# CliffKai/BridgeLang

Hardware: AMD Instinct MI355X
Metric: action-seqs/sec (7-DoF, 224px) openvla-7b bf16 (higher is better)
Workload: dtype bf16; 1 GPU; openvla-7b bf16 inference (BASELINE configs[1]): batch 16 synthetic 224px frames + 32-token prompts per GPU, predict_action = vision towers + projector + Llama prefill S=288 + 6 cached decode steps, greedy; 7 batches in flight: per step one batch is submitted (vision+prefill) while decode iteration g of the batch submitted g steps earlier, g = 1..6, runs as ONE merged 96-row pass over the weights ; batch_per_gpu=16, prompt_len=32, seq_len=288, replicas=1, hip_graph=True, pipeline_depth=7

## Files before the change

### bridgelang_amd/csrc/gemm_bf16.hip

```cpp
#include "gemm_common.h"
#include <stdlib.h>

namespace bl_gemm_bf16_impl {
using namespace blgemm;

typedef __attribute__((ext_vector_type(4))) short s16x4_t;

template <int EPI>
__global__ __launch_bounds__(256) void gemm128_kernel(GemmArgs p) {
#if defined(__HIP_DEVICE_COMPILE__)
  constexpr int BM = 128, BN = 128, WN = 2, NWAVE = 4;
  constexpr int TM = 64, TN = 64, MT = 4, NT = 4;
  constexpr int A_BYTES = BM * ROW_BYTES, BUF_BYTES = A_BYTES + BN * ROW_BYTES;
  extern __shared__ __attribute__((aligned(16))) char smem[];

  int tm, tn;
  tile_coords(p, tm, tn);
  const int m0 = tm * BM, n0 = tn * BN;
  const int tid = threadIdx.x, lane = tid & 63;
  const int wave = __builtin_amdgcn_readfirstlane(tid >> 6);
  const int wm = wave / WN, wn = wave % WN;
  const int kt32 = p.K >> 5;

  const unsigned a_bytes = (unsigned)min((long)p.M * p.lda * 2, 0xffffffffL);
// ... 631 lines not shown
  constexpr int A_BYTES = BM * ROW_BYTES, DUMMY = A_BYTES, W_OFF = A_BYTES + 4096, STAGE = W_OFF + 32768;
  extern __shared__ __attribute__((aligned(16))) char smem[];
  int tm, tn;
  tile_coords(p, tm, tn);
  const int m0 = tm * BM, n0 = tn * BN;
  const int tid = threadIdx.x, lane = tid & 63;
  const int wave = __builtin_amdgcn_readfirstlane(tid >> 6);
  const int wm = wave >> 2, wn = wave & 3;
  const int l15 = lane & 15, lg = lane >> 4;
  const int kt32 = p.K >> 5, nk = p.K / BK;

  const unsigned a_bytes = (unsigned)min((long)p.M * p.lda * 2, 0xffffffffL);
  const unsigned w_bytes = (unsigned)min((long)p.N * p.K * 2, 0xffffffffL);
  const int prow = lane >> 3, pchunk = (lane & 7) ^ prow;
  unsigned voffA[5];
  int ldsA[5];
#pragma unroll
  for (int j = 0; j < 5; ++j) {
    const int pi = wave + 8 * j;
    voffA[j] = (unsigned)(((long)(m0 + pi * 8 + prow) * p.lda) * 2 + pchunk * 16);
    ldsA[j] = pi < 36 ? pi * 1024 : DUMMY + (pi - 36) * 1024;
  }
  const unsigned a4_bytes = wave < 4 ? a_bytes : 0u;
  unsigned voffW[2];
#pragma unroll
  for (int q = 0; q < 2; ++q) voffW[q] = (unsigned)((long)(n0 / 16 + 2 * wave + q) * kt32 * 1024 + lane * 16);
  const int ldsW = W_OFF + 2 * wave * 2048;
#define BL_RS(PTR, BYTES) __builtin_amdgcn_make_buffer_rsrc((void*)(PTR), 0, (BYTES), 0x00020000)
#define ISSUE_A(J, TILE)                                                                                  \
  do {                                                                                                    \
    const int t__ = (TILE);                                                                               \
    const __amdgpu_buffer_rsrc_t rs__ = BL_RS(p.A, t__ < nk ? ((J) < 4 ? a_bytes : a4_bytes) : 0u);       \
    BL_GLDS(rs__, smem + (t__ & 1) * STAGE + ldsA[J], voffA[J], t__ * 128);                               \
  } while (0)
#define ISSUE_W(Q, KS, TILE)                                                                              \
  do {                                                                                                    \
    const int t__ = (TILE);                                                                               \
    const __amdgpu_buffer_rsrc_t rs__ = BL_RS(p.W, t__ < nk ? w_bytes : 0u);                              \
    BL_GLDS(rs__, smem + (t__ & 1) * STAGE + ldsW + (Q) * 2048 + (KS) * 1024, voffW[Q] + (KS) * 1024, t__ * 2048); \
  } while (0)
  const int cb0 = (lg ^ (lane & 7)) << 4;
  const int offX = (wm * 144 + l15) * ROW_BYTES;
  const int offY = W_OFF + wn * 8192 + lane * 16;
#define READ_X(T3, SB)                                                                                    \
  _Pragma("unroll") for (int i = 0; i < 3; ++i) {                                                         \
    X[i * 2] = *(const bf16x8_t*)((SB) + offX + (3 * (T3) + i) * 2048 + cb0);                             \
    X[i * 2 + 1] = *(const bf16x8_t*)((SB) + offX + (3 * (T3) + i) * 2048 + (cb0 ^ 64));                  \
  }
#define READ_Y(DST, NH, SB)                                                                               \
  _Pragma("unroll") for (int j = 0; j < 2; ++j) {                                                         \
    DST[j * 2] = *(const bf16x8_t*)((SB) + offY + (2 * (NH) + j) * 2048);                                 \
    DST[j * 2 + 1] = *(const bf16x8_t*)((SB) + offY + (2 * (NH) + j) * 2048 + 1024);                      \
  }
#define MMA(YR, T3, NH)                                                                                   \
  _Pragma("unroll") for (int ks = 0; ks < 2; ++ks)                                                        \
    _Pragma("unroll") for (int j = 0; j < 2; ++j)                                                         \
      _Pragma("unroll") for (int i = 0; i < 3; ++i)                                                       \
        acc[2 * (NH) + j][3 * (T3) + i] = __builtin_amdgcn_mfma_f32_16x16x32_bf16(                        \
            YR[j * 2 + ks], X[i * 2 + ks], acc[2 * (NH) + j][3 * (T3) + i], 0, 0, 0);
#define PHASE(T3)                                                                                         \
  do {                                                                                                    \
    __builtin_amdgcn_s_setprio(1);                                                                        \
    MMA(Ya, T3, 0)                                                                                        \
    MMA(Yb, T3, 1)                                                                                        \
    __builtin_amdgcn_s_setprio(0);                                                                        \
  } while (0)
#define BAR()                                                                                             \
  do {                                                                                                    \
    __builtin_amdgcn_s_barrier();                                                                         \
    __builtin_amdgcn_sched_barrier(0);                                                                    \
  } while (0)
#define WAIT_LGKM() asm volatile("s_waitcnt lgkmcnt(0)" ::: "memory")
#define WAIT_VM4_LGKM() asm volatile("s_waitcnt vmcnt(4) lgkmcnt(0)" ::: "memory")
#define SLOT0(SC, T) do { READ_X(0, SC); READ_Y(Ya, 0, SC); READ_Y(Yb, 1, SC); __builtin_amdgcn_sched_barrier(0); ISSUE_A(0, (T) + 1); ISSUE_A(1, (T) + 1); WAIT_LGKM(); } while (0)
#define SLOT1(SC, T) do { READ_X(1, SC); __builtin_amdgcn_sched_barrier(0); ISSUE_A(2, (T) + 1); ISSUE_A(3, (T) + 1); ISSUE_A(4, (T) + 1); WAIT_LGKM(); } while (0)
#define SLOT2(SC, T) do { READ_X(2, SC); __builtin_amdgcn_sched_barrier(0); ISSUE_W(0, 0, (T) + 2); ISSUE_W(0, 1, (T) + 2); ISSUE_W(1, 0, (T) + 2); ISSUE_W(1, 1, (T) + 2); WAIT_VM4_LGKM(); } while (0)
#define BL_EPILOGUE()                                                                                     \
  do {                                                                                                    \
    asm volatile("s_waitcnt vmcnt(0)" ::: "memory");                                                      \
    const int ncol__[4] = {n0 + wn * 64 + lg * 4, n0 + wn * 64 + 16 + lg * 4, n0 + wn * 64 + 32 + lg * 4,      \
                           n0 + wn * 64 + 48 + lg * 4};                                                   \
    epilogue_tile<EPI, 4, 9>(p, m0 + wm * 144 + l15, ncol__, m0 + 288, n0 + 256, acc);                    \
  } while (0)

  f32x4_t acc[4][9];
#pragma unroll
  for (int i = 0; i < 4; ++i)
#pragma unroll
    for (int j = 0; j < 9; ++j) acc[i][j] = (f32x4_t){0.f, 0.f, 0.f, 0.f};
  bf16x8_t X[6], Ya[4], Yb[4];
  char* const S0 = smem;
  char* const S1 = smem + STAGE;

  ISSUE_A(0, 0); ISSUE_A(1, 0); ISSUE_A(2, 0); ISSUE_A(3, 0); ISSUE_A(4, 0);
  ISSUE_W(0, 0, 0); ISSUE_W(0, 1, 0); ISSUE_W(1, 0, 0); ISSUE_W(1, 1, 0);
  ISSUE_W(0, 0, 1); ISSUE_W(0, 1, 1); ISSUE_W(1, 0, 1); ISSUE_W(1, 1, 1);
  asm volatile("s_waitcnt vmcnt(4)" ::: "memory");
  BAR();
  if (wm == 0) {
    SLOT0(S0, 0);
    BAR();
    for (int t = 0; t < nk; t += 2) {
      PHASE(0); BAR();   SLOT1(S0, t); BAR();
      PHASE(1); BAR();   SLOT2(S0, t); BAR();
      PHASE(2); BAR();   SLOT0(S1, t + 1); BAR();
      PHASE(0); BAR();   SLOT1(S1, t + 1); BAR();
      PHASE(1); BAR();   SLOT2(S1, t + 1); BAR();
      PHASE(2); BAR();   SLOT0(S0, t + 2); BAR();
    }
    BL_EPILOGUE();
    return;
  }
  BAR();
  for (int t = 0; t < nk; t += 2) {
    SLOT0(S0, t); BAR();       PHASE(0); BAR();
    SLOT1(S0, t); BAR();       PHASE(1); BAR();
    SLOT2(S0, t); BAR();       PHASE(2); BAR();
    SLOT0(S1, t + 1); BAR();   PHASE(0); BAR();
    SLOT1(S1, t + 1); BAR();   PHASE(1); BAR();
    SLOT2(S1, t + 1); BAR();   PHASE(2); BAR();
  }
  BL_EPILOGUE();
#undef BL_RS
#undef ISSUE_A
#undef ISSUE_W
#undef READ_X
#undef READ_Y
#undef MMA
#undef PHASE
#undef BAR
#undef WAIT_LGKM
#undef WAIT_VM4_LGKM
#undef SLOT0
#undef SLOT1
#undef SLOT2
#undef BL_EPILOGUE
#endif
}

template <int EPI, bool TN = false>
__global__ __launch_bounds__(512) void gemm256s_kernel(GemmArgs p) {
#if defined(__HIP_DEVICE_COMPILE__)
  constexpr int BM = 256, BN = 256;
  constexpr int STAGE = 65536, W_OFF = 32768;
  extern __shared__ __attribute__((aligned(16))) char smem[];

  int tm, tn;
  const int nk_all = TN ? (p.K + BK - 1) / BK : p.K / BK;
  int kt_begin = 0, nk = nk_all;
  const int ptiles = p.splitk > 1 ? 0 : p.ptiles;
  int vb = blockIdx.x;
  if (p.splitk > 1) {
    lin_to_tile(p, p.tail_base + blockIdx.x / p.splitk, tm, tn);
    const int slice = blockIdx.x % p.splitk;
    kt_begin = (int)(((long)slice * nk_all) / p.splitk) & ~1;
    nk = slice + 1 == p.splitk ? nk_all : ((int)(((long)(slice + 1) * nk_all) / p.splitk) & ~1);
  } else if (ptiles > 0) {
    tile_coords_v(p, vb, ptiles, tm, tn);
  } else {
    tile_coords(p, tm, tn);
  }
  int m0 = tm * BM, n0 = tn * BN;
  const int tid = threadIdx.x, lane = tid & 63;
  const int wave = __builtin_amdgcn_readfirstlane(tid >> 6);
  const int wm = wave >> 2, wn = wave & 3;
  const int l15 = lane & 15, lg = lane >> 4;
  const int kt32 = p.K >> 5;

  const long a_total = TN ? ((long)(p.K - 1) * p.lda + p.M) * 2 : (long)p.M * p.lda * 2;
  const long w_total = TN ? ((long)(p.K - 1) * p.ldw + p.N) * 2 : (long)p.N * p.K * 2;
  const int kstepX = TN ? (int)(64 * p.lda * 2) : 128, kstepY = TN ? (int)(64 * p.ldw * 2) : 2048;
#define TILE_A_OFF(M0) (TN ? (long)(M0) * 2 : (long)(M0) * p.lda * 2)
#define TILE_W_OFF(N0) (TN ? (long)(N0) * 2 : (long)((N0) / 16) * (p.K >> 5) * 1024)
  const char* Acur = (const char*)p.A + TILE_A_OFF(m0);
  const char* Wcur = (const char*)p.W + TILE_W_OFF(n0);
  unsigned a_bytes = (unsigned)min(a_total - TILE_A_OFF(m0), 0xffffffffL);
  unsigned w_bytes = (unsigned)min(w_total - TILE_W_OFF(n0), 0xffffffffL);
  const char* Anext = Acur; const char* Wnext = Wcur;
  unsigned a_bytes_next = 0u, w_bytes_next = 0u;
  int m0_next = 0, n0_next = 0;
#define BL_NEXT_TILE()                                                                      \
  do {                                                                                      \
    a_bytes_next = 0u; w_bytes_next = 0u;                                                   \
    if (ptiles > 0 && vb + (int)gridDim.x < ptiles) {                                       \
      int tm__, tn__;                                                                       \
      tile_coords_v(p, vb + (int)gridDim.x, ptiles, tm__, tn__);                            \
      m0_next = tm__ * BM; n0_next = tn__ * BN;                                             \
      Anext = (const char*)p.A + TILE_A_OFF(m0_next);                                       \
      Wnext = (const char*)p.W + TILE_W_OFF(n0_next);                                       \
      a_bytes_next = (unsigned)min(a_total - TILE_A_OFF(m0_next), 0xffffffffL);             \
      w_bytes_next = (unsigned)min(w_total - TILE_W_OFF(n0_next), 0xffffffffL);             \
    }                                                                                       \
  } while (0)
  BL_NEXT_TILE();

  const int prow = lane >> 3, pchunk = (lane & 7) ^ prow;
  unsigned voffX[2][2], voffY[2][2];
  int ldsX[2][2], ldsY[2];
  if constexpr (!TN) {
#pragma unroll
    for (int mh = 0; mh < 2; ++mh)
#pragma unroll
      for (int j = 0; j < 2; ++j) {
        const int pi = 2 * wave + j, row0 = (pi >> 3) * 128 + mh * 64 + (pi & 7) * 8;
        voffX[mh][j] = (unsigned)(((long)(row0 + prow) * p.lda) * 2 + pchunk * 16);
        ldsX[mh][j] = row0 * ROW_BYTES;
      }
#pragma unroll
    for (int nh = 0; nh < 2; ++nh) {
      const int nt = (wave >> 1) * 4 + 2 * nh + (wave & 1);
      voffY[nh][0] = (unsigned)((long)nt * kt32 * 1024 + lane * 16);
      voffY[nh][1] = voffY[nh][0] + 1024;
      ldsY[nh] = W_OFF + nt * 2048;
    }
  } else {
#pragma unroll
    for (int mh = 0; mh < 2; ++mh)
#pragma unroll
      for (int j = 0; j < 2; ++j) {
        const int pi = 2 * wave + j, t = (pi & 7) * 8 + prow, pos = lane & 7;
        const int c = ((((pos >> 1) ^ ((t >> 1) & 3)) << 1) | (pos & 1));
        voffX[mh][j] = (unsigned)((long)t * p.lda * 2 + (long)((pi >> 3) * 128 + mh * 64) * 2 + c * 16);
        ldsX[mh][j] = ((pi >> 3) * 128 + mh * 64 + (pi & 7) * 8) * ROW_BYTES;
      }
#pragma unroll
    for (int nh = 0; nh < 2; ++nh) {
#pragma unroll
      for (int j = 0; j < 2; ++j) {
        const int t = (2 * wave + j) * 4 + (lane >> 4), pos = lane & 15;
        const int c = ((((pos >> 1) ^ (t & 7)) << 1) | (pos & 1));
        voffY[nh][j] = (unsigned)((long)t * p.ldw * 2 + (long)(nh * 128) * 2 + c * 16);
      }
      ldsY[nh] = W_OFF + nh * 16384 + wave * 2048;
    }
  }
#define BL_RS(PTR, BYTES) __builtin_amdgcn_make_buffer_rsrc((void*)(PTR), 0, (BYTES), 0x00020000)
#define ISSUE_X(MH, TILE)                                                                   \
  do {                                                                                      \
    const int t__ = (TILE);                                                                 \
    const bool nx__ = t__ >= nk;                         \
    const int tt__ = nx__ ? t__ - nk : t__;                                                 \
    const __amdgpu_buffer_rsrc_t rs__ = BL_RS(nx__ ? Anext : Acur, nx__ ? a_bytes_next : a_bytes); \
    char* b__ = smem + (t__ & 1) * STAGE;                                                   \
    BL_GLDS(rs__, b__ + ldsX[MH][0], voffX[MH][0], tt__ * kstepX);                             \
    BL_GLDS(rs__, b__ + ldsX[MH][1], voffX[MH][1], tt__ * kstepX);                             \
  } while (0)
#define ISSUE_Y(NH, TILE)                                                                   \
  do {                                                                                      \
    const int t__ = (TILE);                                                                 \
    const bool nx__ = t__ >= nk;                                                            \
    const int tt__ = nx__ ? t__ - nk : t__;                                                 \
    const __amdgpu_buffer_rsrc_t rs__ = BL_RS(nx__ ? Wnext : Wcur, nx__ ? w_bytes_next : w_bytes); \
    char* b__ = smem + (t__ & 1) * STAGE;                                                   \
    BL_GLDS(rs__, b__ + ldsY[NH], voffY[NH][0], tt__ * kstepY);                               \
    BL_GLDS(rs__, b__ + ldsY[NH] + 1024, voffY[NH][1], tt__ * kstepY);                        \
  } while (0)
  const int cb0 = (lg ^ (lane & 7)) << 4;
  const int offX = (wm * 128 + l15) * ROW_BYTES;
  const int offY = W_OFF + wn * 8192 + lane * 16;
  const int trX = (wm * 128) * ROW_BYTES + (4 * lg + (l15 >> 2)) * 128 + (l15 & 3) * 8, swX = ((lg & 1) << 1) | (l15 >> 3);
  const int trY = W_OFF + (4 * lg + (l15 >> 2)) * 256 + (l15 & 3) * 8, swY = ((lg & 1) << 2) | (l15 >> 2);
  const unsigned ldsbase = (unsigned)(size_t)LDS_PTR(smem);
#define BL_TR(DST, ADDR, OFF) asm volatile("ds_read_b64_tr_b16 %0, %1 offset:%2" : "=v"(DST) : "v"(ADDR), "n"(OFF))
#define BL_PIN(R) asm volatile("" : "+v"(R))
#define READ_X(DST, MH, SB)                                                                             \
  do {                                                                                                  \
    if constexpr (!TN) {                                                                                \
      _Pragma("unroll") for (int i = 0; i < 4; ++i) {                                                   \
        DST[i * 2] = *(const bf16x8_t*)((SB) + offX + (MH) * 8192 + i * 2048 + cb0);                    \
        DST[i * 2 + 1] = *(const bf16x8_t*)((SB) + offX + (MH) * 8192 + i * 2048 + (cb0 ^ 64));        \
      }                                                                                                 \
    } else {                                                                                            \
      _Pragma("unroll") for (int i = 0; i < 4; ++i) {                                                   \
        const unsigned a__ = ldsbase + (unsigned)((SB) - smem) + trX + ((i ^ swX) << 5);                \
        BL_TR(DST##2[i * 4 + 0], a__, (MH) * 8192);                                                     \
        BL_TR(DST##2[i * 4 + 1], a__, (MH) * 8192 + 2048);                                              \
        BL_TR(DST##2[i * 4 + 2], a__, (MH) * 8192 + 4096);                                              \
        BL_TR(DST##2[i * 4 + 3], a__, (MH) * 8192 + 4096 + 2048);                                       \
      }                                                                                                 \
    }                                                                                                   \
  } while (0)
#define READ_Y(DST, NH, SB)                                                                             \
  do {                                                                                                  \
    if constexpr (!TN) {                                                                                \
      _Pragma("unroll") for (int j = 0; j < 2; ++j) {                                                   \
        DST[j * 2] = *(const bf16x8_t*)((SB) + offY + (2 * (NH) + j) * 2048);                           \
        DST[j * 2 + 1] = *(const bf16x8_t*)((SB) + offY + (2 * (NH) + j) * 2048 + 1024);                \
      }                                                                                                 \
    } else {                                                                                            \
      _Pragma("unroll") for (int j = 0; j < 2; ++j) {                                                   \
        const unsigned a__ = ldsbase + (unsigned)((SB) - smem) + trY + (((wn * 2 + j) ^ swY) << 5);     \
        BL_TR(DST##2[j * 4 + 0], a__, (NH) * 16384);                                                    \
        BL_TR(DST##2[j * 4 + 1], a__, (NH) * 16384 + 4096);                                             \
        BL_TR(DST##2[j * 4 + 2], a__, (NH) * 16384 + 8192);                                             \
        BL_TR(DST##2[j * 4 + 3], a__, (NH) * 16384 + 8192 + 4096);                                      \
      }                                                                                                 \
    }                                                                                                   \
  } while (0)
#define BL_FRAG(R2, F, KS)                                                                              \
  __builtin_bit_cast(bf16x8_t, ((u32x4_t){R2[(F) * 4 + 2 * (KS)][0], R2[(F) * 4 + 2 * (KS)][1],         \
                                          R2[(F) * 4 + 2 * (KS) + 1][0], R2[(F) * 4 + 2 * (KS) + 1][1]}))
#define MMA(XR, YR, MH, NH)                                                                             \
  do {                                                                                                  \
    if constexpr (TN) {                                                                                 \
      _Pragma("unroll") for (int q = 0; q < 16; ++q) BL_PIN(XR##2[q]);                                  \
      _Pragma("unroll") for (int q = 0; q < 8; ++q) BL_PIN(YR##2[q]);                                   \
    }                                                                                                   \
    __builtin_amdgcn_s_setprio(1);                                                                      \
    _Pragma("unroll") for (int ks = 0; ks < 2; ++ks)                                                    \
      _Pragma("unroll") for (int j = 0; j < 2; ++j)                                                     \
        _Pragma("unroll") for (int i = 0; i < 4; ++i) {                                                 \
          if constexpr (TN)                                                                             \
            acc[2 * (NH) + j][4 * (MH) + i] = __builtin_amdgcn_mfma_f32_16x16x32_bf16(                  \
                BL_FRAG(YR##2, j, ks), BL_FRAG(XR##2, i, ks), acc[2 * (NH) + j][4 * (MH) + i], 0, 0, 0); \
          else                                                                                          \
            acc[2 * (NH) + j][4 * (MH) + i] = __builtin_amdgcn_mfma_f32_16x16x32_bf16(                  \
                YR[j * 2 + ks], XR[i * 2 + ks], acc[2 * (NH) + j][4 * (MH) + i], 0, 0, 0);              \
        }                                                                                               \
    __builtin_amdgcn_s_setprio(0);                                                                      \
  } while (0)
#define BAR()                                   \
  do {                                          \
    __builtin_amdgcn_s_barrier();               \
    __builtin_amdgcn_sched_barrier(0);          \
  } while (0)
#define WAIT_VM8() asm volatile("s_waitcnt vmcnt(8)" ::: "memory")
#define WAIT_VM10_LGKM() asm volatile("s_waitcnt vmcnt(10) lgkmcnt(0)" ::: "memory")
#define WAIT_LGKM() asm volatile("s_waitcnt lgkmcnt(0)" ::: "memory")
#define ISSUE_READ(I, R) do { R; __builtin_amdgcn_sched_barrier(0); I; } while (0)
#define ISSUE_Q0(T) ISSUE_X(1, (T) + 1)
#define ISSUE_Q1(T) ISSUE_Y(0, (T) + 2)
#define ISSUE_Q2(T) ISSUE_X(0, (T) + 2)
#define ISSUE_Q3(T) ISSUE_Y(1, (T) + 2)
#define BL_EPILOGUE()                                                                                     \
  do {                                                                                                    \
    if (a_bytes_next == 0u && w_bytes_next == 0u)    \
      asm volatile("s_waitcnt vmcnt(0)" ::: "memory");                                                    \
    if (p.splitk > 1) {                                                                                   \
      long off__ = ((long)blockIdx.x * 32 * 512 + tid) * 4;                                               \
      asm volatile("" : "+v"(off__));    \
      float* dst = p.slab + off__;                                                                        \
      _Pragma("unroll") for (int i = 0; i < 4; ++i)                                                       \
        _Pragma("unroll") for (int j = 0; j < 8; ++j) *(f32x4_t*)(dst + (long)(i * 8 + j) * 512 * 4) = acc[i][j]; \
    } else {                                                                                              \
      int ncol__[4];                                                                                      \
      _Pragma("unroll") for (int i = 0; i < 4; ++i)                                                       \
        ncol__[i] = TN ? n0 + (i >> 1) * 128 + wn * 32 + (i & 1) * 16 + lg * 4 : n0 + wn * 64 + i * 16 + lg * 4; \
      epilogue_tile<EPI, 4, 8>(p, m0 + wm * 128 + l15, ncol__, m0 + 256, n0 + 256, acc);                  \
    }                                                                                                     \
  } while (0)

#define BL_ADVANCE()                                                                                      \
  do {                                                                                                    \
    vb += (int)gridDim.x;                                                                                 \
    m0 = m0_next; n0 = n0_next; Acur = Anext; Wcur = Wnext; a_bytes = a_bytes_next; w_bytes = w_bytes_next; \
    BL_NEXT_TILE();                                                                                       \
    _Pragma("unroll") for (int i = 0; i < 4; ++i)                                                         \
      _Pragma("unroll") for (int j = 0; j < 8; ++j) acc[i][j] = (f32x4_t){0.f, 0.f, 0.f, 0.f};            \
  } while (0)

  f32x4_t acc[4][8];
#pragma unroll
  for (int i = 0; i < 4; ++i)
#pragma unroll
    for (int j = 0; j < 8; ++j) acc[i][j] = (f32x4_t){0.f, 0.f, 0.f, 0.f};
  bf16x8_t X[8], Ya[4], Yb[4];
  u32x2_t X2[16], Ya2[8], Yb2[8];
  char* const S0 = smem;
  char* const S1 = smem + STAGE;
  const int t0 = kt_begin;

  ISSUE_Y(0, t0); ISSUE_X(0, t0); ISSUE_Y(1, t0); ISSUE_X(1, t0); ISSUE_Y(0, t0 + 1); ISSUE_X(0, t0 + 1); ISSUE_Y(1, t0 + 1);
  asm volatile("s_waitcnt vmcnt(10)" ::: "memory");
  BAR();
  READ_Y(Ya, 0, S0);

  if (wm == 0) {
    READ_X(X, 0, S0);
    WAIT_LGKM();
    BAR();
    for (;;) {
    for (int t = t0; t < nk; t += 2) {
      MMA(X, Ya, 0, 0); WAIT_VM8(); BAR();   ISSUE_READ(ISSUE_Q0(t), READ_Y(Yb, 1, S0)); WAIT_LGKM(); BAR();
      MMA(X, Yb, 0, 1); WAIT_VM8(); BAR();   ISSUE_READ(ISSUE_Q1(t), READ_X(X, 1, S0));  WAIT_LGKM(); BAR();
      MMA(X, Yb, 1, 1); WAIT_VM8(); BAR();   ISSUE_READ(ISSUE_Q2(t), READ_Y(Yb, 0, S1)); WAIT_LGKM(); BAR();
      MMA(X, Ya, 1, 0); WAIT_VM8(); BAR();   ISSUE_READ(ISSUE_Q3(t), READ_X(X, 0, S1));  WAIT_LGKM(); BAR();
      MMA(X, Yb, 0, 0); WAIT_VM8(); BAR();   ISSUE_READ(ISSUE_Q0(t + 1), READ_Y(Ya, 1, S1)); WAIT_LGKM(); BAR();
      MMA(X, Ya, 0, 1); WAIT_VM8(); BAR();   ISSUE_READ(ISSUE_Q1(t + 1), READ_X(X, 1, S1));  WAIT_LGKM(); BAR();
      MMA(X, Ya, 1, 1); WAIT_VM8(); BAR();   ISSUE_READ(ISSUE_Q2(t + 1), READ_Y(Ya, 0, S0)); WAIT_LGKM(); BAR();
      MMA(X, Yb, 1, 0); WAIT_VM8(); BAR();   ISSUE_READ(ISSUE_Q3(t + 1), READ_X(X, 0, S0));  WAIT_LGKM(); BAR();
    }
    const bool more = a_bytes_next != 0u;
    BL_EPILOGUE();
    if (!more) break;
    BL_ADVANCE();
    }
    return;
  }
  WAIT_LGKM();
  BAR();
  for (;;) {
  for (int t = t0; t < nk; t += 2) {
    ISSUE_READ(ISSUE_Q0(t), READ_X(X, 0, S0));  WAIT_VM10_LGKM(); BAR();   MMA(X, Ya, 0, 0); BAR();
    ISSUE_READ(ISSUE_Q1(t), READ_Y(Yb, 1, S0)); WAIT_VM10_LGKM(); BAR();   MMA(X, Yb, 0, 1); BAR();
    ISSUE_READ(ISSUE_Q2(t), READ_X(X, 1, S0));  WAIT_VM10_LGKM(); BAR();   MMA(X, Yb, 1, 1); BAR();
    ISSUE_READ(ISSUE_Q3(t), READ_Y(Yb, 0, S1)); WAIT_VM10_LGKM(); BAR();   MMA(X, Ya, 1, 0); BAR();
    ISSUE_READ(ISSUE_Q0(t + 1), READ_X(X, 0, S1));  WAIT_VM10_LGKM(); BAR();   MMA(X, Yb, 0, 0); BAR();
    ISSUE_READ(ISSUE_Q1(t + 1), READ_Y(Ya, 1, S1)); WAIT_VM10_LGKM(); BAR();   MMA(X, Ya, 0, 1); BAR();
    ISSUE_READ(ISSUE_Q2(t + 1), READ_X(X, 1, S1));  WAIT_VM10_LGKM(); BAR();   MMA(X, Ya, 1, 1); BAR();
    ISSUE_READ(ISSUE_Q3(t + 1), READ_Y(Ya, 0, S0)); WAIT_VM10_LGKM(); BAR();   MMA(X, Yb, 1, 0); BAR();
  }
  const bool more = a_bytes_next != 0u;
  BL_EPILOGUE();
  if (!more) break;
  BL_ADVANCE();
  }
#undef BL_EPILOGUE
#undef BL_ADVANCE
#undef BL_NEXT_TILE
#undef TILE_A_OFF
#undef TILE_W_OFF
#undef ISSUE_X
#undef ISSUE_Y
#undef READ_X
#undef READ_Y
#undef BL_TR
#undef BL_PIN
#undef BL_FRAG
#undef MMA
#undef BAR
#undef WAIT_VM8
#undef WAIT_VM10_LGKM
#undef WAIT_LGKM
#undef ISSUE_READ
#undef ISSUE_Q0
#undef ISSUE_Q1
#undef ISSUE_Q2
#undef ISSUE_Q3
#endif
}

template <int EPI, bool TN = false>
__global__ __launch_bounds__(512) void gemm_splitk_reduce_kernel(GemmArgs p) {
  int tm, tn;
  const int tile_local = blockIdx.x >> 5, idx = blockIdx.x & 31, i = idx >> 3, j = idx & 7;
  lin_to_tile(p, p.tail_base + tile_local, tm, tn);
  const int tid = threadIdx.x, lane = tid & 63, wave = tid >> 6;
  const int wm = wave >> 2, wn = wave & 3, l15 = lane & 15, lg = lane >> 4;
  f32x4_t sum = {0.f, 0.f, 0.f, 0.f};
  for (int s = 0; s < p.splitk; ++s)
    sum += *(const f32x4_t*)(p.slab + (((long)(tile_local * p.splitk + s) * 32 + idx) * 512 + tid) * 4);
  epilogue_store4<EPI>(p, tm * 256 + wm * 128 + j * 16 + l15,
                       TN ? tn * 256 + (i >> 1) * 128 + wn * 32 + (i & 1) * 16 + lg * 4 : tn * 256 + wn * 64 + i * 16 + lg * 4, sum);
}

#define BL_RING8(X, EPI, BM, BN) X(kid(KN_RING8, BM, BN), (gemm_ring8_kernel<EPI, BM, BN, 4>))
#define BL_MID(X, EPI, MB, NB, SK) X(kid(KN_MID, MB, NB, SK), (gemm_mid_kernel<EPI, MB, NB, SK>))
#define BL_MID2(X, EPI, NT, NST) X(kid(KN_MID2, NT, NST), (gemm_mid2_kernel<EPI, NT, NST>))
#define BL_ROWS_STREAM(X, ID, EPI, NWV, SK) X(kid(ID, NWV, SK), (gemm_rows_stream_kernel<EPI, NWV, SK>))
#define BL_TILE_KERNELS(X, EPI)                                                                                       \
  X(kid(KN_GEMM128), (gemm128_kernel<EPI>)) X(kid(KN_GEMM288S), (gemm288s_kernel<EPI>))                               \
  X(kid(KN_GEMM256S), (gemm256s_kernel<EPI>)) X(kid(KN_TILE_REDUCE), (gemm_splitk_reduce_kernel<EPI>))                \
  X(kid(KN_SLAB_REDUCE), (gemm128_splitk_reduce_kernel<EPI>))                                                         \
  BL_RING8(X, EPI, 160, 128) BL_RING8(X, EPI, 128, 128) BL_RING8(X, EPI, 128, 64) BL_RING8(X, EPI, 64, 64)            \
  BL_MID(X, EPI, 2, 4, 0) BL_MID(X, EPI, 4, 4, 0) BL_MID(X, EPI, 5, 4, 0) BL_MID(X, EPI, 2, 1, 0) BL_MID(X, EPI, 4, 1, 0) \
  BL_MID(X, EPI, 5, 1, 0) BL_MID2(X, EPI, 1, 3) BL_MID2(X, EPI, 4, 3) BL_MID2(X, EPI, 2, 2)
#define BL_ROWS_KERNELS(X, EPI)                                                                                       \
  BL_ROWS_STREAM(X, KN_ROWS_STREAM, EPI, 8, 8) BL_ROWS_STREAM(X, KN_ROWS_STREAM, EPI, 6, 8)                           \
  BL_ROWS_STREAM(X, KN_ROWS_STREAM_HALVES, BL_EPI_NONE, 8, 4) BL_MID(X, EPI, 2, 4, 8) BL_MID(X, EPI, 2, 4, 2)         \
  X(kid(KN_TREE_REDUCE), (gemm_rows_tree_reduce_kernel<EPI>))
#define BL_TN_KERNELS(X, EPI) \
  X(kid(KN_GEMM256S, 1), (gemm256s_kernel<BL_EPI_F32, true>)) X(kid(KN_TILE_REDUCE, 1), (gemm_splitk_reduce_kernel<BL_EPI_F32, true>))

BL_KERNEL_FAMILY(TileKernels, BL_TILE_KERNELS)
BL_KERNEL_FAMILY(RowsKernels, BL_ROWS_KERNELS)
BL_KERNEL_FAMILY(TnKernels, BL_TN_KERNELS)

}
using namespace bl_gemm_bf16_impl;

extern "C" int bl_gemm_last_form(void) { return gemm_last_form(); }

extern "C" int bl_gemm_bf16(const bl_gemm_desc* d, void* stream) {
  gemm_last_form() = 0;
  GemmArgs a;
  const int rc = fill_gemm_args(d, a);
  if (rc != BL_OK) return rc;
  if (d->a_norm_weight) return BL_E_ARG;
  const GemmPlan plan = plan_gemm(gemm_shape(a));
  return with_epilogue<ALL_EPIS>(d->epilogue, [&](auto epi) {
    return launch_plan<TileKernels<decltype(epi)::value>>(plan, a, (hipStream_t)stream);
  });
}

extern "C" int bl_gemm_skinny_rows_bf16(const bl_gemm_desc* d, void* stream) {
  gemm_last_form() = 0;
  GemmArgs a;
  const int rc = fill_gemm_args(d, a);
  if (rc != BL_OK) return rc;
  if (d->M > 128 || (d->K % 256) || d->a_norm_weight) return BL_E_SHAPE;
  if (d->out_group) return BL_E_ARG;
  const char* e_on = getenv("BL_ROWS_STREAM");
  const GemmPlan plan = plan_rows(gemm_shape(a, e_on ? atoi(e_on) != 0 : true));
  return with_epilogue<SKINNY_EPIS>(d->epilogue, [&](auto epi) {
    return launch_plan<RowsKernels<decltype(epi)::value>>(plan, a, (hipStream_t)stream);
  });
}

extern "C" int bl_gemm_tn_bf16(const bl_gemm_desc* d, void* stream) {
  gemm_last_form() = 0;
  if (!d || !d->A || !d->W || !d->C) return BL_E_ARG;
  if (d->epilogue != BL_EPI_F32 || d->out_group || d->a_norm_weight) return BL_E_ARG;
  if (d->M <= 0 || d->N <= 0 || d->K <= 0 || (d->M % 8) || (d->N % 8)) return BL_E_SHAPE;
  if ((d->lda % 8) || (d->ldw % 8) || (d->ldc % 4) || d->lda < d->M || d->ldw < d->N || d->ldc < d->N) return BL_E_ALIGN;
  if (!bl_aligned16(d->A) || !bl_aligned16(d->W) || (((uintptr_t)d->C) & 15)) return BL_E_ALIGN;
  if ((long)d->K * d->lda * 2 >= (1L << 31) || (long)d->K * d->ldw * 2 >= (1L << 31)) return BL_E_SHAPE;
  GemmArgs a = {};
  a.A = d->A; a.W = d->W; a.C = d->C;
  a.lda = d->lda; a.ldw = d->ldw; a.ldc = d->ldc;
  a.M = d->M; a.N = d->N; a.K = d->K;
  a.tail_base = -1;
  a.slab = (float*)d->workspace; a.slab_bytes = d->workspace_bytes; a.splitk = 1;
  return launch_plan<TnKernels<BL_EPI_F32>>(plan_gemm_tn(gemm_shape(a)), a, (hipStream_t)stream);
}
```

Before: 280.3 action-seqs/s.

## Restructure 256x256 GEMM ping-pong schedule into four coarser phases per k-pair

```diff
diff --git a/bridgelang_amd/csrc/gemm_bf16.hip b/bridgelang_amd/csrc/gemm_bf16.hip
--- a/bridgelang_amd/csrc/gemm_bf16.hip
+++ b/bridgelang_amd/csrc/gemm_bf16.hip
@@ -957,11 +957,6 @@
                                           R2[(F) * 4 + 2 * (KS) + 1][0], R2[(F) * 4 + 2 * (KS) + 1][1]}))
 #define MMA(XR, YR, MH, NH)                                                                             \
   do {                                                                                                  \
-    if constexpr (TN) {                                                                                 \
-      _Pragma("unroll") for (int q = 0; q < 16; ++q) BL_PIN(XR##2[q]);                                  \
-      _Pragma("unroll") for (int q = 0; q < 8; ++q) BL_PIN(YR##2[q]);                                   \
-    }                                                                                                   \
-    __builtin_amdgcn_s_setprio(1);                                                                      \
     _Pragma("unroll") for (int ks = 0; ks < 2; ++ks)                                                    \
       _Pragma("unroll") for (int j = 0; j < 2; ++j)                                                     \
         _Pragma("unroll") for (int i = 0; i < 4; ++i) {                                                 \
@@ -972,21 +967,41 @@
             acc[2 * (NH) + j][4 * (MH) + i] = __builtin_amdgcn_mfma_f32_16x16x32_bf16(                  \
                 YR[j * 2 + ks], XR[i * 2 + ks], acc[2 * (NH) + j][4 * (MH) + i], 0, 0, 0);              \
         }                                                                                               \
+  } while (0)
+#define PHASE(YFIRST, YSECOND, MH, NFIRST, NSECOND)                                                     \
+  do {                                                                                                  \
+    if constexpr (TN) {                                                                                 \
+      _Pragma("unroll") for (int q = 0; q < 16; ++q) BL_PIN(X2[q]);                                     \
+      _Pragma("unroll") for (int q = 0; q < 8; ++q) { BL_PIN(Ya2[q]); BL_PIN(Yb2[q]); }                 \
+    }                                                                                                   \
+    __builtin_amdgcn_s_setprio(1);                                                                      \
+    MMA(X, YFIRST, MH, NFIRST);                                                                         \
+    MMA(X, YSECOND, MH, NSECOND);                                                                       \
     __builtin_amdgcn_s_setprio(0);                                                                      \
   } while (0)
+#define PHASE0() PHASE(Ya, Yb, 0, 0, 1)
+#define PHASE1() PHASE(Yb, Ya, 1, 1, 0)
 #define BAR()                                   \
   do {                                          \
     __builtin_amdgcn_s_barrier();               \
     __builtin_amdgcn_sched_barrier(0);          \
   } while (0)
-#define WAIT_VM8() asm volatile("s_waitcnt vmcnt(8)" ::: "memory")
-#define WAIT_VM10_LGKM() asm volatile("s_waitcnt vmcnt(10) lgkmcnt(0)" ::: "memory")
-#define WAIT_LGKM() asm volatile("s_waitcnt lgkmcnt(0)" ::: "memory")
-#define ISSUE_READ(I, R) do { R; __builtin_amdgcn_sched_barrier(0); I; } while (0)
-#define ISSUE_Q0(T) ISSUE_X(1, (T) + 1)
-#define ISSUE_Q1(T) ISSUE_Y(0, (T) + 2)
-#define ISSUE_Q2(T) ISSUE_X(0, (T) + 2)
-#define ISSUE_Q3(T) ISSUE_Y(1, (T) + 2)
+#define WAIT_VM8_LGKM() asm volatile("s_waitcnt vmcnt(8) lgkmcnt(0)" ::: "memory")
+#define WAIT_VM4_LGKM() asm volatile("s_waitcnt vmcnt(4) lgkmcnt(0)" ::: "memory")
+#define SLOT_READS(R) do { R; __builtin_amdgcn_sched_barrier(0); } while (0)
+#define SLOT_ISSUES(I) do { I; } while (0)
+#define SLOT0(SC, T)                                                             \
+  do {                                                                           \
+    SLOT_READS(READ_X(X, 0, SC); READ_Y(Ya, 0, SC); READ_Y(Yb, 1, SC));          \
+    SLOT_ISSUES(ISSUE_X(1, (T) + 1); ISSUE_Y(1, (T) + 1));                       \
+    WAIT_VM8_LGKM();                                                             \
+  } while (0)
+#define SLOT1(SC, T)                                                             \
+  do {                                                                           \
+    SLOT_READS(READ_X(X, 1, SC));                                                \
+    SLOT_ISSUES(ISSUE_Y(0, (T) + 2); ISSUE_X(0, (T) + 2));                       \
+    WAIT_VM4_LGKM();                                                             \
+  } while (0)
 #define BL_EPILOGUE()                                                                                     \
   do {                                                                                                    \
     if (a_bytes_next == 0u && w_bytes_next == 0u)    \
@@ -1025,25 +1040,19 @@
   char* const S1 = smem + STAGE;
   const int t0 = kt_begin;
 
-  ISSUE_Y(0, t0); ISSUE_X(0, t0); ISSUE_Y(1, t0); ISSUE_X(1, t0); ISSUE_Y(0, t0 + 1); ISSUE_X(0, t0 + 1); ISSUE_Y(1, t0 + 1);
-  asm volatile("s_waitcnt vmcnt(10)" ::: "memory");
+  ISSUE_Y(0, t0); ISSUE_X(0, t0); ISSUE_X(1, t0); ISSUE_Y(1, t0); ISSUE_Y(0, t0 + 1); ISSUE_X(0, t0 + 1);
+  asm volatile("s_waitcnt vmcnt(4)" ::: "memory");
   BAR();
-  READ_Y(Ya, 0, S0);
 
   if (wm == 0) {
-    READ_X(X, 0, S0);
-    WAIT_LGKM();
+    SLOT0(S0, t0);
     BAR();
     for (;;) {
     for (int t = t0; t < nk; t += 2) {
-      MMA(X, Ya, 0, 0); WAIT_VM8(); BAR();   ISSUE_READ(ISSUE_Q0(t), READ_Y(Yb, 1, S0)); WAIT_LGKM(); BAR();
-      MMA(X, Yb, 0, 1); WAIT_VM8(); BAR();   ISSUE_READ(ISSUE_Q1(t), READ_X(X, 1, S0));  WAIT_LGKM(); BAR();
-      MMA(X, Yb, 1, 1); WAIT_VM8(); BAR();   ISSUE_READ(ISSUE_Q2(t), READ_Y(Yb, 0, S1)); WAIT_LGKM(); BAR();
-      MMA(X, Ya, 1, 0); WAIT_VM8(); BAR();   ISSUE_READ(ISSUE_Q3(t), READ_X(X, 0, S1));  WAIT_LGKM(); BAR();
-      MMA(X, Yb, 0, 0); WAIT_VM8(); BAR();   ISSUE_READ(ISSUE_Q0(t + 1), READ_Y(Ya, 1, S1)); WAIT_LGKM(); BAR();
-      MMA(X, Ya, 0, 1); WAIT_VM8(); BAR();   ISSUE_READ(ISSUE_Q1(t + 1), READ_X(X, 1, S1));  WAIT_LGKM(); BAR();
-      MMA(X, Ya, 1, 1); WAIT_VM8(); BAR();   ISSUE_READ(ISSUE_Q2(t + 1), READ_Y(Ya, 0, S0)); WAIT_LGKM(); BAR();
-      MMA(X, Yb, 1, 0); WAIT_VM8(); BAR();   ISSUE_READ(ISSUE_Q3(t + 1), READ_X(X, 0, S0));  WAIT_LGKM(); BAR();
+      PHASE0(); BAR();   SLOT1(S0, t); BAR();
+      PHASE1(); BAR();   SLOT0(S1, t + 1); BAR();
+      PHASE0(); BAR();   SLOT1(S1, t + 1); BAR();
+      PHASE1(); BAR();   SLOT0(S0, t + 2); BAR();
     }
     const bool more = a_bytes_next != 0u;
     BL_EPILOGUE();
@@ -1052,18 +1061,13 @@
     }
     return;
   }
-  WAIT_LGKM();
   BAR();
   for (;;) {
   for (int t = t0; t < nk; t += 2) {
-    ISSUE_READ(ISSUE_Q0(t), READ_X(X, 0, S0));  WAIT_VM10_LGKM(); BAR();   MMA(X, Ya, 0, 0); BAR();
-    ISSUE_READ(ISSUE_Q1(t), READ_Y(Yb, 1, S0)); WAIT_VM10_LGKM(); BAR();   MMA(X, Yb, 0, 1); BAR();
-    ISSUE_READ(ISSUE_Q2(t), READ_X(X, 1, S0));  WAIT_VM10_LGKM(); BAR();   MMA(X, Yb, 1, 1); BAR();
-    ISSUE_READ(ISSUE_Q3(t), READ_Y(Yb, 0, S1)); WAIT_VM10_LGKM(); BAR();   MMA(X, Ya, 1, 0); BAR();
-    ISSUE_READ(ISSUE_Q0(t + 1), READ_X(X, 0, S1));  WAIT_VM10_LGKM(); BAR();   MMA(X, Yb, 0, 0); BAR();
-    ISSUE_READ(ISSUE_Q1(t + 1), READ_Y(Ya, 1, S1)); WAIT_VM10_LGKM(); BAR();   MMA(X, Ya, 0, 1); BAR();
-    ISSUE_READ(ISSUE_Q2(t + 1), READ_X(X, 1, S1));  WAIT_VM10_LGKM(); BAR();   MMA(X, Ya, 1, 1); BAR();
-    ISSUE_READ(ISSUE_Q3(t + 1), READ_Y(Ya, 0, S0)); WAIT_VM10_LGKM(); BAR();   MMA(X, Yb, 1, 0); BAR();
+    SLOT0(S0, t); BAR();       PHASE0(); BAR();
+    SLOT1(S0, t); BAR();       PHASE1(); BAR();
+    SLOT0(S1, t + 1); BAR();   PHASE0(); BAR();
+    SLOT1(S1, t + 1); BAR();   PHASE1(); BAR();
   }
   const bool more = a_bytes_next != 0u;
   BL_EPILOGUE();
@@ -1083,15 +1087,16 @@
 #undef BL_PIN
 #undef BL_FRAG
 #undef MMA
+#undef PHASE
+#undef PHASE0
+#undef PHASE1
 #undef BAR
-#undef WAIT_VM8
-#undef WAIT_VM10_LGKM
-#undef WAIT_LGKM
-#undef ISSUE_READ
-#undef ISSUE_Q0
-#undef ISSUE_Q1
-#undef ISSUE_Q2
-#undef ISSUE_Q3
+#undef WAIT_VM8_LGKM
+#undef WAIT_VM4_LGKM
+#undef SLOT_READS
+#undef SLOT_ISSUES
+#undef SLOT0
+#undef SLOT1
 #endif
 }
 
```

Result: no change. 281.0 action-seqs/s (median of 6 runs) (+0.3%).
